# letitiabanana/PnP-OVSS

Measured on AMD Instinct MI355X. Metric: images/sec (336^2, drop_iter=4, blur+CRF), higher is better.
Workload: dtype bf16x3

## Files before the change

pnp-ovss_amd/csrc/engine.hip:

```cpp
#include <cmath>
#include <cstring>
#include <utility>

#include "engine.h"

using namespace pnp;

namespace {

int alloc_act(pnp_engine* e, Act* a, size_t rows, size_t ld) {
    KCHK(e, dalloc_t(e, &a->hi, rows * ld));
    a->lo = e->x3 ? (char*)a->hi + rows * ld * 2 : nullptr;
    return PNP_OK;
}

bool ends_with(const std::string& s, const char* suf) {
    const size_t n = strlen(suf);
    return s.size() >= n && s.compare(s.size() - n, n, suf) == 0;
}

__global__ void transpose_cast_kernel_f32(const float* __restrict__ in, float* __restrict__ out, int rows, int cols) {
    __shared__ float t[32][33];
    const int bx = blockIdx.x * 32, by = blockIdx.y * 32;
    for (int i = threadIdx.y; i < 32; i += 8) {
        const int r = by + i, c = bx + threadIdx.x;
        t[i][threadIdx.x] = (r < rows && c < cols) ? in[(size_t)r * cols + c] : 0.f;
    }
    __syncthreads();
    for (int i = threadIdx.y; i < 32; i += 8) {
        const int c = bx + i, r = by + threadIdx.x;
        if (r < rows && c < cols) out[(size_t)c * rows + r] = t[threadIdx.x][i];
    }
}

__global__ void feat_to_tok_kernel(const float* __restrict__ src, int ld_src, int n_pad, float* __restrict__ dst, int R, int N) {
    __shared__ float t[32][33];
    const int b = blockIdx.z, r0 = blockIdx.x * 32, t0 = blockIdx.y * 32;
    for (int i = threadIdx.y; i < 32; i += 8) {
        const int r = r0 + i, tok = t0 + threadIdx.x;
        t[i][threadIdx.x] = (r < R && tok < N) ? src[(size_t)r * ld_src + (size_t)b * n_pad + tok] : 0.f;
    }
    __syncthreads();
    for (int i = threadIdx.y; i < 32; i += 8) {
        const int tok = t0 + i, r = r0 + threadIdx.x;
        if (r < R && tok < N) dst[((size_t)b * N + tok) * R + r] = t[threadIdx.x][i];
    }
}
__global__ void tok_to_feat_kernel(const float* __restrict__ src, int ld_src, float* __restrict__ dst, int ld_dst, int n_pad, int R, int N) {
    __shared__ float t[32][33];
    const int b = blockIdx.z, r0 = blockIdx.x * 32, t0 = blockIdx.y * 32;
    for (int i = threadIdx.y; i < 32; i += 8) {
        const int tok = t0 + i, r = r0 + threadIdx.x;
        t[i][threadIdx.x] = (r < R && tok < N) ? src[((size_t)b * N + tok) * ld_src + r] : 0.f;
    }
    __syncthreads();
    for (int i = threadIdx.y; i < 32; i += 8) {
        const int r = r0 + i, tok = t0 + threadIdx.x;
        if (r < R && tok < N) dst[(size_t)r * ld_dst + (size_t)b * n_pad + tok] = t[threadIdx.x][i];
    }
}

__global__ void embed_reuse_kernel(const float* __restrict__ x0, const uint8_t* __restrict__ dropped, const float* __restrict__ bias,
                                   const float* __restrict__ pos, float* __restrict__ x, int rows, int N, int D4) {
    const size_t total = (size_t)rows * D4;
    for (size_t i = (size_t)blockIdx.x * blockDim.x + threadIdx.x; i < total; i += (size_t)gridDim.x * blockDim.x) {
        const int m = (int)(i / D4), c = (int)(i - (size_t)m * D4);
        const int b = m / N, t = m - b * N;
        f32x4 v;
        if (t > 0 && dropped[(size_t)b * (N - 1) + (t - 1)]) {
            const f32x4 bv = reinterpret_cast<const f32x4*>(bias)[c];
            const f32x4 pv = reinterpret_cast<const f32x4*>(pos)[(size_t)t * D4 + c];
#pragma unroll
            for (int e = 0; e < 4; e++) v[e] = __fadd_rn(__fadd_rn(0.0f, bv[e]), pv[e]);
        } else {
            v = reinterpret_cast<const f32x4*>(x0)[i];
        }
        reinterpret_cast<f32x4*>(x)[i] = v;
    }
}

int new_weight(pnp_engine* e, int rows, int cols, bool pair, Weight* w) {
    *w = Weight{nullptr, rows, cols, pair ? 2 : (int)e->esz, pair};
    return dalloc_t(e, &w->p, (size_t)rows * cols);
}
int fill_weight(pnp_engine* e, const float* src32, const Weight& w, int r0, int n) {
    const size_t count = (size_t)n * w.cols;
    return w.pair ? split_f32(src32, w.hi(r0), w.lo(r0), count, 0) : cast_f32(e->bf, src32, w.hi(r0), count, 0);
}
int make_weight(pnp_engine* e, const float* src32, int rows, int cols, bool transpose, Weight* out, bool pair = false) {
    KCHK(e, new_weight(e, transpose ? cols : rows, transpose ? rows : cols, pair, out));
    const float* s = src32;
    float* tmp = nullptr;
// ... 448 lines not shown
            KCHK(e, make_weight(e, st[W_SO], H, H, true, &t.so_wT, e->x3));
        }
    }
    for (int i = 0; i < 2; i++) {
        const float *w = staged(e, std::string(kProj[i]) + ".weight"), *bs = staged(e, std::string(kProj[i]) + ".bias");
        if (!w || !bs) {
            e->proj_E[i] = 0;
            continue;
        }
        KCHK(e, make_weight(e, w, e->proj_E[i], i == 0 ? D : H, false, &e->proj_w[i], e->x3));
        KCHK(e, dalloc(e, &e->proj_b[i], (size_t)e->proj_E[i]));
        HIPCHK(e, hipMemcpy(e->proj_b[i], bs, (size_t)e->proj_E[i] * 4, hipMemcpyDeviceToDevice));
    }
    HIPCHK(e, hipDeviceSynchronize());
    for (auto& b : e->staging) if (b.p) (void)hipFree(b.p);
    e->staging.clear();
    for (auto it = e->named.begin(); it != e->named.end();) {
        if (it->first.rfind("stage:", 0) == 0) it = e->named.erase(it);
        else ++it;
    }
    e->finalized = true;
    return PNP_OK;
}


static int vit_forward_impl(pnp_engine* e, const float* d_images, const uint8_t* d_dropped, int32_t B, void* stream, int embed) {
    if (!e || !d_images) return PNP_ERR_ARG;
    if (!e->finalized) return fail(e, PNP_ERR_STATE, "weights not finalized");
    if (B <= 0 || B > e->c.max_batch) return fail(e, PNP_ERR_ARG, "batch %d out of range (max %d)", B, e->c.max_batch);
    hipStream_t s = (hipStream_t)stream;
    const int D = e->D, N = e->N, M = B * N, F = D * e->c.vit_mlp_ratio, bf = e->bf;
    const int ldv = e->c.max_batch * e->Npad;
    if (embed == 2 && !(e->reuse.vit && e->reuse.images == d_images && e->reuse.B == B)) embed = 0;
    if (embed == 2 && d_dropped) {
        hipLaunchKernelGGL(embed_reuse_kernel, dim3(2048), dim3(256), 0, s, (const float*)e->x0, d_dropped, (const float*)e->patch_b,
                           (const float*)e->pos, e->x, M, N, D / 4);
        KCHK(e, launched());
    } else {
        KCHK(e, patchify(bf, d_images, d_dropped, e->patches, B, e->c.img_size, e->P, s));
        KCHK(e, cls_rows(e->cls, e->pos, e->x, B, N, D, s));
        {
            GemmArgs g = linear(e->patches, 768, e->patch_w, B * e->PP);
            g.bias = e->patch_b; g.resid = e->pos; g.ldr = D; g.out_f32 = e->x; g.ldo = D; g.row_div = e->PP;
            KCHK(e, egemm(e, g, s));
        }
        if (embed == 1) {
            HIPCHK(e, hipMemcpyAsync(e->x0, e->x, (size_t)M * D * sizeof(float), hipMemcpyDeviceToDevice, s));
            e->reuse.images = d_images;
            e->reuse.B = B;
            e->reuse.vit = true;
        }
    }
    const float scale = 1.0f / sqrtf(64.f);
    const int ln = bf | e->x3;
    for (int l = 0; l < e->c.vit_depth; l++) {
        const VitLayerW& w = e->vit[l];
        KCHK(e, layernorm(ln, e->x, w.n1w, w.n1b, e->c.vit_ln_eps, M, D, nullptr, e->xn.hi, nullptr, nullptr, s, e->xn.lo));
        if (bf || e->x3) {
            GemmArgs g = linear(e->xn, D, w.qkv_w, M);
            g.bias = w.qkv_b; g.out_t = e->qk.hi; g.out_lo = e->qk.lo; g.ldo_t = e->ldq;
            KCHK(e, egemm(e, g, s));
            if (e->x3)
                KCHK(e, vit_attention_x3(e->qk.hi, e->qk.lo, e->ldq, D, e->ctx.hi, e->ctx.lo, B, e->c.vit_heads, N, scale, s));
            else
                KCHK(e, vit_attention(bf, e->qk.hi, e->ldq, D, (const char*)e->qk.hi + (size_t)2 * D * e->esz, e->ldq, e->Npad, e->ctx.hi,
                                      B, e->c.vit_heads, N, scale, s));
        } else {
            {
                GemmArgs g = linear(e->xn, D, w.qkv_w, M, 0, 2 * D);
                g.bias = w.qkv_b; g.out_t = e->qk.hi; g.ldo_t = 2 * D;
                KCHK(e, egemm(e, g, s));
            }
            {
                GemmArgs g = linear_t(e->xn, D, w.qkv_w, M, 2 * D, D);
                g.bias = w.qkv_b + 2 * D; g.bias_on_rows = 1; g.out_t = e->vt; g.ldo_t = ldv; g.col_div = N; g.col_pad = e->Npad;
                KCHK(e, egemm(e, g, s));
            }
            KCHK(e, vit_attention(bf, e->qk.hi, 2 * D, D, e->vt, ldv, e->Npad, e->ctx.hi, B, e->c.vit_heads, N, scale, s));
        }
        {
            GemmArgs g = linear(e->ctx, D, w.proj_w, M);
            g.bias = w.proj_b; g.resid = e->x; g.ldr = D; g.out_f32 = e->x; g.ldo = D;
            KCHK(e, egemm(e, g, s));
        }
        KCHK(e, layernorm(ln, e->x, w.n2w, w.n2b, e->c.vit_ln_eps, M, D, nullptr, e->xn.hi, nullptr, nullptr, s, e->xn.lo));
        {
            GemmArgs g = linear(e->xn, D, w.fc1_w, M);
            g.bias = w.fc1_b; g.mode = GEMM_EPI_GELU; g.out_t = e->h1.hi; g.out_lo = e->h1.lo; g.ldo_t = F;
            KCHK(e, egemm(e, g, s));
        }
        {
            GemmArgs g = linear(e->h1, F, w.fc2_w, M);
            g.bias = w.fc2_b; g.resid = e->x; g.ldr = D; g.out_f32 = e->x; g.ldo = D;
            KCHK(e, egemm(e, g, s));
        }
    }
    KCHK(e, layernorm(ln, e->x, e->vnorm_w, e->vnorm_b, e->c.vit_ln_eps, M, D, e->emb32, e->embT.hi, nullptr, nullptr, s, e->embT.lo));
    return pnp_cross_kv(e, B, stream);
}
extern "C" int pnp_vit_forward(pnp_engine* e, const float* d_images, const uint8_t* d_dropped, int32_t B, void* stream) {
    if (e) e->reuse.vit = false;
    return vit_forward_impl(e, d_images, d_dropped, B, stream, 0);
}

extern "C" int pnp_cross_kv(pnp_engine* e, int32_t B, void* stream) {
    if (!e) return PNP_ERR_ARG;
    if (!e->finalized) return fail(e, PNP_ERR_STATE, "weights not finalized");
    if (B <= 0 || B > e->c.max_batch) return fail(e, PNP_ERR_ARG, "batch %d out of range (max %d)", B, e->c.max_batch);
    hipStream_t s = (hipStream_t)stream;
    const int D = e->D, N = e->N, M = B * N;
    const int ldv = e->c.max_batch * e->Npad;
    const int H = e->H, TL = e->TL, SL = e->SL, nVn = TL - SL, nKt = TL - SL - 1;
    auto out = [&](GemmArgs& g, void* p, int ld) {
        if (e->x3) { g.out_f32 = (float*)p; g.ldo = ld; }
        else { g.out_t = p; g.ldo_t = ld; }
    };
    {
        GemmArgs g = linear(e->embT, D, e->ck_w, M);
        g.bias = e->ck_b; out(g, e->Knat, TL * H);
        KCHK(e, egemm(e, g, s));
    }
    {
        GemmArgs g = linear_t(e->embT, D, e->cv_w, M);
        g.bias = e->cv_b; g.bias_on_rows = 1; out(g, e->Vt, ldv); g.col_div = N; g.col_pad = e->Npad;
        KCHK(e, egemm(e, g, s));
    }
    if (e->x3) {
        hipLaunchKernelGGL(feat_to_tok_kernel, dim3((nVn * H + 31) / 32, (N + 31) / 32, B), dim3(32, 8), 0, s,
                           (const float*)e->Vt + (size_t)SL * H * ldv, ldv, e->Npad, (float*)e->Vnat, nVn * H, N);
        KCHK(e, launched());
        if (nKt > 0) {
            hipLaunchKernelGGL(tok_to_feat_kernel, dim3((nKt * H + 31) / 32, (N + 31) / 32, B), dim3(32, 8), 0, s,
                               (const float*)e->Knat + (size_t)(SL + 1) * H, TL * H, (float*)e->Kt, ldv, e->Npad, nKt * H, N);
            KCHK(e, launched());
        }
        return PNP_OK;
    }
    {
        GemmArgs g = linear(e->embT, D, e->cv_w, M, SL * H, nVn * H);
        g.bias = e->cv_b + (size_t)SL * H; g.out_t = e->Vnat; g.ldo_t = nVn * H;
        KCHK(e, egemm(e, g, s));
    }
    if (nKt > 0) {
        GemmArgs g = linear_t(e->embT, D, e->ck_w, M, (SL + 1) * H, nKt * H);
        g.bias = e->ck_b + (size_t)(SL + 1) * H; g.bias_on_rows = 1; g.out_t = e->Kt; g.ldo_t = ldv; g.col_div = N; g.col_pad = e->Npad;
        KCHK(e, egemm(e, g, s));
    }
    return PNP_OK;
}

static int text_layer(pnp_engine* e, int i, const int64_t* d_mask, int32_t ld, int32_t B, int32_t L, bool cross, bool self_in_place,
                      hipStream_t s) {
    const int H = e->H, I = e->I, TL = e->TL, R = B * L, bf = e->bf, N = e->N;
    const int ldv = e->c.max_batch * e->Npad;
    const TextLayerW& w = e->txt[i];
    TextLayerA& a = e->ta[i];
    const float* h = i ? e->ta[i - 1].h_out : e->h0;
    const void* hT = i ? e->ta[i - 1].h_outT : e->h0T;
    const bool keep_p = cross && i >= e->SL;
    auto keep = [&](float* p) -> float* { return cross ? p : nullptr; };
    if (!self_in_place) {
        {
            GemmArgs g = linear(hT, H, w.qkv_w, R);
            g.bias = w.qkv_b; g.out_t = a.qkv; g.ldo_t = 3 * H;
            KCHK(e, egemm(e, g, s));
        }
// ... 264 lines not shown
    if (!e || !d_images || !d_ids || !d_mask || !d_g0) return PNP_ERR_ARG;
    if (drop_iter < 1) return fail(e, PNP_ERR_ARG, "drop_iter must be >= 1");
    if (drop_iter == 1)
        return pnp_compute_gradcam_layer(e, d_images, nullptr, d_ids, d_mask, ld, B, L, layer, head, d_g0, d_logits, stream);
    if (!d_agg || !d_picks) return PNP_ERR_ARG;
    hipStream_t s = (hipStream_t)stream;
    HIPCHK(e, hipMemsetAsync(e->dropped, 0, (size_t)B * e->PP, s));
    for (int it = 0; it < drop_iter; it++) {
        int r = compute_gradcam_impl(e, d_images, e->dropped, d_ids, d_mask, ld, B, L, layer, head, e->G, d_logits, stream, it == 0 ? 1 : 2);
        if (r) return r;
        r = pnp_drop_step(e, e->G, d_g0, d_agg, e->dropped, d_picks, it, B, L - 1, npick, drop_iter * npick, stream);
        if (r) return r;
    }
    return PNP_OK;
}


extern "C" int pnp_get_buffer(pnp_engine* e, const char* name, void** d_ptr, size_t* bytes) {
    if (!e || !name || !d_ptr || !bytes) return PNP_ERR_ARG;
    const std::string n(name);
    const size_t B = e->c.max_batch, L = e->c.max_text_len;
    auto set = [&](void* ptr, size_t b) { *d_ptr = ptr; *bytes = b; return PNP_OK; };
    if (n == "image_embeds") return set(e->emb32, B * e->N * (size_t)e->D * 4);
    if (n == "image_embeds_t") return set(e->embT.hi, B * e->N * (size_t)e->D * e->esz);
    if (n == "x") return set(e->x, B * e->N * (size_t)e->D * 4);
    if (n == "P") return set(e->ta[e->grad_layer >= 0 ? e->grad_layer : e->SL].Pc, B * e->nh * L * (size_t)e->Nst * 4);
    if (n == "dP") return set(e->dPc, B * e->nh * L * (size_t)e->Nst * 4);
    if (n == "text_hidden") return set(e->ta[e->TL - 1].h_out, B * L * (size_t)e->H * 4);
    if (n == "h_last") return set(e->ta[e->TL - 1].h_out, B * L * (size_t)e->H * 4);
    if (n == "dropped") return set(e->dropped, B * (size_t)e->PP);
    if (n == "P_last" && e->ta[e->TL - 1].Pc) return set(e->ta[e->TL - 1].Pc, B * e->nh * L * (size_t)e->Nst * 4);
    if (n == "Kt" && e->Kt) return set(e->Kt, (size_t)(e->TL - e->SL - 1) * e->H * B * e->Npad * e->esz);
    if (n == "Vt") return set(e->Vt, (size_t)e->TL * e->H * B * e->Npad * e->esz);
    if (n == "dq_xattn") return set(e->dqc, B * L * (size_t)e->H * e->esz);
    if (n == "dctx_xattn") return set(e->dctxc, B * L * (size_t)e->H * e->esz);
    if (post_get_buffer(e, n, d_ptr, bytes)) return PNP_OK;
    return fail(e, PNP_ERR_ARG, "unknown buffer %s", name);
}

extern "C" size_t pnp_allocated_bytes(const pnp_engine* e) { return e ? e->alloc_bytes : 0; }

extern "C" int pnp_profile_enable(pnp_engine* e, int32_t on) {
    if (!e) return PNP_ERR_ARG;
    if (!e->gemm_prof) {
        if (!on) {
            e->crf_prof.on = false;
            return PNP_OK;
        }
        e->gemm_prof = new GemmProfile();
    }
    GemmProfile& pf = *e->gemm_prof;
    pf.on = on != 0;
    pf.period = on > 1 ? on : 1;
    pf.seq = 0;
    pf.used = 0;
    pf.launches = 0;
    pf.flops = 0;
    e->crf_prof.on = on != 0;
    e->crf_prof.used = 0;
    e->crf_prof.launches = 0;
    e->crf_prof.work = 0;
    e->crf_prof.lattice = 0;
    return PNP_OK;
}

extern "C" int pnp_profile_read_stage(pnp_engine* e, int32_t stage, int64_t* launches, double* work, double* ms) {
// ... 48 lines not shown
                              void* d_out_t, int32_t ldo_t, int32_t mode, void* stream) {
    GemmArgs g = G_(d_A, lda, d_B, ldb, M, N, K);
    g.bias = d_bias; g.resid = d_resid; g.ldr = ldr; g.out_f32 = d_out_f32; g.ldo = ldo; g.out_t = d_out_t; g.ldo_t = ldo_t;
    g.mode = mode ? GEMM_EPI_GELU : GEMM_EPI_LINEAR;
    return gemm_nt(bf, g, (hipStream_t)stream);
}

extern "C" int pnp_op_split(const float* d_in, void* d_hi, void* d_lo, int64_t n, void* stream) {
    if (!d_in || !d_hi || !d_lo || n <= 0) return PNP_ERR_ARG;
    return split_f32(d_in, d_hi, d_lo, (size_t)n, (hipStream_t)stream);
}

extern "C" int pnp_op_gemm_x3(const void* d_A_hi, const void* d_A_lo, int32_t lda, const void* d_B_hi, const void* d_B_lo,
                              int32_t ldb, int32_t M, int32_t N, int32_t K, const float* d_bias, int32_t bias_on_rows,
                              const float* d_resid, int32_t ldr, float* d_out_f32, int32_t ldo, void* d_out_hi, void* d_out_lo,
                              int32_t ldo_t, int32_t gelu, int32_t col_div, int32_t col_pad, void* stream) {
    if (!d_A_hi || !d_A_lo || !d_B_hi || !d_B_lo) return PNP_ERR_ARG;
    GemmArgs g = G_(d_A_hi, lda, d_B_hi, ldb, M, N, K);
    g.A_lo = d_A_lo; g.B_lo = d_B_lo;
    g.bias = d_bias; g.bias_on_rows = bias_on_rows; g.resid = d_resid; g.ldr = ldr; g.out_f32 = d_out_f32; g.ldo = ldo;
    g.out_t = d_out_hi; g.out_lo = d_out_lo; g.ldo_t = ldo_t; g.col_div = col_div; g.col_pad = col_pad;
    g.mode = gelu ? GEMM_EPI_GELU : GEMM_EPI_LINEAR;
    g.sk = streamk_mode() ? streamk_ws_default() : nullptr;
    return gemm_nt(1, g, (hipStream_t)stream);
}

extern "C" int pnp_set_tuning(const char* key, int32_t value) {
    if (!key) return PNP_ERR_ARG;
    if (!strcmp(key, "streamk")) {
        if (value < 0 || value > 2) return PNP_ERR_ARG;
        set_streamk_mode(value);
        return PNP_OK;
    }
    if (!strcmp(key, "text_rows")) {
        if (value < 0 || value > 4) return PNP_ERR_ARG;
        set_text_rows(value);
        return PNP_OK;
    }
    if (!strcmp(key, "gemm_stamps")) {
        if (value < 0 || value > 1) return PNP_ERR_ARG;
        return gemm_set_stamps(value);
    }
    return PNP_ERR_ARG;
}

extern "C" int pnp_streamk_status(pnp_engine* e, int64_t* launches, uint32_t* gave_up) {
    if (!launches || !gave_up) return PNP_ERR_ARG;
    StreamKWs* ws = e ? &e->sk_ws : streamk_ws_default();
    *launches = ws ? ws->launches : 0;
    *gave_up = 0;
    if (!ws || !ws->part) return PNP_OK;
    if (e) HIPCHK(e, hipSetDevice(e->c.device));
    if (hipDeviceSynchronize() != hipSuccess) return PNP_ERR_HIP;
    return streamk_ws_timeouts(ws, gave_up);
}

extern "C" int pnp_op_gemm_x3a(const float* d_A, int32_t lda, const void* d_B_hi, const void* d_B_lo, int32_t ldb, int32_t M,
                               int32_t N, int32_t K, const float* d_bias, const float* d_resid, int32_t ldr, float* d_out_f32,
                               int32_t ldo, int32_t mode, float* d_aux, int32_t ld_aux, void* stream) {
    if (!d_A || !d_B_hi || !d_B_lo || !d_out_f32 || mode < 0 || mode > 2) return PNP_ERR_ARG;
    GemmArgs g = G_(d_A, lda, d_B_hi, ldb, M, N, K);
    g.B_lo = d_B_lo; g.a_f32 = 1;
    g.bias = d_bias; g.resid = d_resid; g.ldr = ldr; g.out_f32 = d_out_f32; g.ldo = ldo;
    g.mode = mode; g.aux = d_aux; g.ld_aux = ld_aux;
    return gemm_nt(0, g, (hipStream_t)stream);
}
// ... 157 lines not shown
```

pnp-ovss_amd/csrc/kernels.h:

```cpp
#pragma once
#include <hip/hip_runtime.h>
#include <stdint.h>
#include <stddef.h>
#include "gemm.h"

namespace pnp {

struct PostDesc {
    int H, W, K, C, has_bg, pix0;
    int Kp;
    int G, Kg;
    size_t off;
    size_t qoff;
    size_t voff[2];
};

struct alignas(16) CrfEntry {
    uint32_t pixel;
    float w;
    float nr;
    uint32_t pad;
};

struct alignas(16) CrfNbr8 {
    int ia, id;
    int pa, pd;
    int aa, ad;
    int da, dd;
};

struct CrfLattice {
    int D1;
    int which;
    size_t cap;
    float* bary;
    uint32_t* vals;
    CrfEntry* ent;
    int* offset;
    int* seg_start;
    int* seg_lo;
    int* seg_hi;
    uint64_t* ukeys;
    int* idbase;
    int* n1;
    int* n2;
    CrfNbr8* nbr8;
};

int patchify(int bf, const float* img, const uint8_t* dropped, void* out, int B, int S, int P, hipStream_t s);
int cls_rows(const float* cls, const float* pos, float* x, int B, int N, int D, hipStream_t s);
int layernorm(int bf, const float* x, const float* w, const float* b, float eps, int rows, int D, float* y, void* yt,
              float* xhat, float* rstd, hipStream_t s, void* yt_lo = nullptr);
int vit_attention(int bf, const void* qk, int ld_qk, int D, const void* vt, int ld_vt, int Npad, void* ctx, int B,
                  int H, int N, float scale, hipStream_t s, void* ctx_lo = nullptr);

int vit_attention_x3(const void* qkv_hi, const void* qkv_lo, int ld_qk, int D, void* ctx_hi, void* ctx_lo, int B, int H, int N,
                     float scale, hipStream_t s);

int text_embed(const int64_t* ids, int ld_ids, const float* word, const float* pos, float* out, int B, int L, int H,
               int enc_id, int vocab, hipStream_t s);
int text_self_attn(int bf, const void* qkv, const int64_t* mask, int ld_mask, void* ctx, float* probs, float* scratch, int B, int L,
                   int H, hipStream_t s);
void set_text_rows(int n);
int text_self_attn_bwd(int bf, const void* qkv, const float* dctx, const float* probs, float* ds_scratch, void* dqkv,
                       int B, int L, int H, hipStream_t s);
int xattn(int bf, int mode, const void* a1, int ld1, const void* a2t, int ld2, int Npad, const void* x, int ldx,
          void* out, int ldo, float* pbuf, int Nst, int B, int L, int N, int nheads, hipStream_t s);
int layernorm_bwd(int bf, const float* dy, const float* w, const float* xhat, const float* rstd, int rows, int D,
                  float* dx, void* dxt, hipStream_t s);
int itm_head(const float* hlast, const float* w, const float* bias, float* logits, int B, int L, int H, hipStream_t s);
int itm_grad_seed(const float* w, float* dh, int B, int L, int H, hipStream_t s);
int cast_f32(int bf, const float* in, void* out, size_t n, hipStream_t s);
int split_f32(const float* in, void* hi, void* lo, size_t n, hipStream_t s);

int l2_normalize_rows(float* x, int rows, int E, float eps, hipStream_t s);
int itc_similarity(const float* img, const float* txt, float* sim, int B, int T, int E, hipStream_t s);
int cast_rows_bf16(const float* in, int ld_in, void* out, int rows, int K, hipStream_t s);

int gradcam_gather(const float* P, const float* dP, const int64_t* mask, int ld_mask, float* out, int B, int nheads,
                   int head, int L, int Nst, int PP, hipStream_t s);
int drop_step(const float* G, float* g0, float* agg, uint8_t* dropped, int32_t* picks, int iter, int B, int T, int PP,
              int npick, int max_picks, hipStream_t s);
int merge_tokens(const float* src, const int32_t* cls_off, const int32_t* tok_idx, const int32_t* cls_div,
                 const int32_t* img_cls_off, float* out, int B, int T, int PP, int Cmax, hipStream_t s);
int threshold_maps(const float* merged, const int32_t* img_cls_off, float* out, float threshold, int B, int PP, int Cmax,
                   hipStream_t s);
int upsample_maps(const float* src, const PostDesc* desc, float* maps, int B, int P, int Cmax, int maxHW, hipStream_t s);
int minmax_normalize(float* maps, const PostDesc* desc, float* stats, int B, int Kmax, int maxHW, int class_channels_only,
                     hipStream_t s);
int background_channel(float* maps, const PostDesc* desc, int B, int maxHW, hipStream_t s);
// ... 69 lines not shown
```

pnp-ovss_amd/csrc/vit_kernels.hip:

```cpp
#include "common.h"
#include "kernels.h"

namespace pnp {

template <typename T>
__global__ void patchify_kernel(const float* __restrict__ img, const uint8_t* __restrict__ dropped,
                                T* __restrict__ out, int B, int S, int P) {
    const int idx = blockIdx.x * blockDim.x + threadIdx.x;
    const int total = B * P * P * 3 * 16;
    if (idx >= total) return;
    const int i = idx & 15;
    const int c = (idx >> 4) % 3;
    const int m = idx / 48;
    const int b = m / (P * P), p = m - b * P * P;
    const int py = p / P, px = p - py * P;
    T* o = out + (size_t)m * 768 + c * 256 + i * 16;
    const bool drop = dropped && dropped[m];
    const float* src = img + (((size_t)b * 3 + c) * S + (py * 16 + i)) * S + px * 16;
#pragma unroll
    for (int v = 0; v < 4; v++) {
        f32x4 x = drop ? f32x4{0.f, 0.f, 0.f, 0.f} : *reinterpret_cast<const f32x4*>(src + v * 4);
#pragma unroll
        for (int e = 0; e < 4; e++) o[v * 4 + e] = from_f32<T>(x[e]);
    }
}

__global__ void cls_rows_kernel(const float* __restrict__ cls, const float* __restrict__ pos,
                                float* __restrict__ x, int B, int N, int D) {
    const int idx = blockIdx.x * blockDim.x + threadIdx.x;
    if (idx >= B * D) return;
    const int b = idx / D, d = idx - b * D;
    x[(size_t)b * N * D + d] = cls[d] + pos[d];
// ... 168 lines not shown
                Frag<T> fv;
                lds_frag_acc_order<ROWB>(fv, Vs, dt * 16 + r, u, q);
                mma16(acc_o[dt], fv, fp);
            }
        }
    }
#undef PNP_LOAD_TILE
    if (q_valid) {
        const float inv = 1.0f / l_run;
        T* o = ctx + (row0 + qrow) * D + h * 64 + q * 4;
#pragma unroll
        for (int dt = 0; dt < 4; dt++) {
            if constexpr (sizeof(T) == 2) {
                bf16x4 pk = {(bf16)(acc_o[dt][0] * inv), (bf16)(acc_o[dt][1] * inv), (bf16)(acc_o[dt][2] * inv),
                             (bf16)(acc_o[dt][3] * inv)};
                *reinterpret_cast<bf16x4*>(o + dt * 16) = pk;
            } else {
                f32x4 ov = acc_o[dt] * inv;
                if (ctx_hi) {
                    const size_t off = (row0 + qrow) * D + h * 64 + q * 4 + dt * 16;
                    const bf16x4 ph = {(bf16)ov[0], (bf16)ov[1], (bf16)ov[2], (bf16)ov[3]};
                    const bf16x4 pl = {(bf16)(ov[0] - (float)ph[0]), (bf16)(ov[1] - (float)ph[1]), (bf16)(ov[2] - (float)ph[2]),
                                       (bf16)(ov[3] - (float)ph[3])};
                    *reinterpret_cast<bf16x4*>(ctx_hi + off) = ph;
                    *reinterpret_cast<bf16x4*>(ctx_lo + off) = pl;
                } else {
                    *reinterpret_cast<f32x4*>(o + dt * 16) = ov;
                }
            }
        }
    }
}

__global__ __launch_bounds__(512) void vit_attn32_kernel(const bf16* __restrict__ qk, int ld_qk, int D,
                                                         const bf16* __restrict__ vt, int ld_vt, int Npad,
                                                         bf16* __restrict__ ctx, int N, float scale, int nqw) {
    constexpr int ROWB = 128, TILE = 64 * ROWB;
    __shared__ __attribute__((aligned(16))) char ring[2][2 * TILE];

    const int tid = threadIdx.x, lane = tid & 63, wave = __builtin_amdgcn_readfirstlane(tid >> 6);
    const int nwaves = blockDim.x >> 6;
    const int l32 = lane & 31, hi = lane >> 5;
    const int b = blockIdx.z, h = blockIdx.y;
    const size_t row0 = (size_t)b * N;
    const int qw = blockIdx.x * nwaves + wave;
    int qrow = qw * 32 + l32;
    const bool q_valid = qw < nqw && qrow < N;
    qrow = qrow < N ? qrow : N - 1;

    bf16x8 fq[4];
    {
        const bf16* qp = qk + (row0 + qrow) * ld_qk + h * 64 + hi * 8;
#pragma unroll
        for (int ks = 0; ks < 4; ks++) fq[ks] = *reinterpret_cast<const bf16x8*>(qp + ks * 16);
    }

    const char* kbase = reinterpret_cast<const char*>(qk + row0 * ld_qk + D + h * 64);
    const char* vbase = reinterpret_cast<const char*>(vt + row0 * ld_vt + h * 64);
    const int prow = lane >> 3, pc = lane & 7;
    auto issue_tile = [&](int t) {
        char* dst = ring[t & 1];
        for (int p = wave; p < 16; p += nwaves) {
            const int row = (p & 7) * 8 + prow;
            const int sc = pc ^ ((row >> 1) & 7);
            int key = t * 64 + row;
            key = key < N ? key : N - 1;
            const char* src = p < 8 ? kbase + (size_t)key * ld_qk * 2 + sc * 16 : vbase + (size_t)key * ld_vt * 2 + sc * 16;
            __builtin_amdgcn_global_load_lds((const __attribute__((address_space(1))) void*)src,
                                             (__attribute__((address_space(3))) void*)(dst + p * 1024), 16, 0, 0);
        }
    };

    f32x16 o[2];
#pragma unroll
    for (int i = 0; i < 2; i++)
#pragma unroll
        for (int e = 0; e < 16; e++) o[i][e] = 0.f;
    float m_run = -INFINITY, l_run = 0.f;
// ... 64 lines not shown
#pragma unroll
            for (int dt = 0; dt < 2; dt++) {
                typedef __attribute__((ext_vector_type(4))) short s16x4;
                s16x4 part[2];
#pragma unroll
                for (int u = 0; u < 2; u++) {
                    const int key = 16 * j + 8 * u + 4 * hi + tq;
                    const int col = dt * 32 + grp_d + 4 * tp;
                    const char* a = Vs + key * ROWB + ((((col >> 3)) ^ ((key >> 1) & 7)) << 4) + (col & 7) * 2;
                    part[u] = __builtin_amdgcn_ds_read_tr16_b64_v4i16((__attribute__((address_space(3))) s16x4*)a);
                }
                const bf16x4 lo = __builtin_bit_cast(bf16x4, part[0]), hh = __builtin_bit_cast(bf16x4, part[1]);
                const bf16x8 fv = {lo[0], lo[1], lo[2], lo[3], hh[0], hh[1], hh[2], hh[3]};
                o[dt] = __builtin_amdgcn_mfma_f32_32x32x16_bf16(fv, fp[j], o[dt], 0, 0, 0);
            }
    }
    l_run += __shfl_xor(l_run, 32, 64);
    if (q_valid) {
        const float inv = 1.0f / l_run;
        bf16* op = ctx + (row0 + qrow) * D + h * 64 + hi * 4;
#pragma unroll
        for (int dt = 0; dt < 2; dt++)
#pragma unroll
            for (int g4 = 0; g4 < 4; g4++) {
                const bf16x4 pk = {(bf16)(o[dt][g4 * 4] * inv), (bf16)(o[dt][g4 * 4 + 1] * inv), (bf16)(o[dt][g4 * 4 + 2] * inv),
                                   (bf16)(o[dt][g4 * 4 + 3] * inv)};
                *reinterpret_cast<bf16x4*>(op + dt * 32 + g4 * 8) = pk;
            }
    }
}

__global__ __launch_bounds__(768) void vit_attn32_x3_kernel(const bf16* __restrict__ qk, const bf16* __restrict__ qk_lo, int ld_qk, int D,
                                                            const bf16* __restrict__ vt, const bf16* __restrict__ vt_lo, int ld_vt,
                                                            bf16* __restrict__ ctx, bf16* __restrict__ ctx_lo, int N, float scale, int nqw) {
    constexpr int ROWB = 128, TILE = 64 * ROWB;
    __shared__ __attribute__((aligned(16))) char ring[2][4 * TILE];

    const int tid = threadIdx.x, lane = tid & 63, wave = __builtin_amdgcn_readfirstlane(tid >> 6);
    const int nwaves = blockDim.x >> 6;
    const int l32 = lane & 31, hi = lane >> 5;
    const int b = blockIdx.z, h = blockIdx.y;
    const size_t row0 = (size_t)b * N;
    const int qw = blockIdx.x * nwaves + wave;
    int qrow = qw * 32 + l32;
    const bool q_valid = qw < nqw && qrow < N;
    qrow = qrow < N ? qrow : N - 1;

    bf16x8 fq[4], fql[4];
    {
        const size_t off = (row0 + qrow) * ld_qk + h * 64 + hi * 8;
#pragma unroll
        for (int ks = 0; ks < 4; ks++) {
            fq[ks] = *reinterpret_cast<const bf16x8*>(qk + off + ks * 16);
            fql[ks] = *reinterpret_cast<const bf16x8*>(qk_lo + off + ks * 16);
        }
    }
    const size_t koff = (row0 * ld_qk + D + h * 64) * 2, voff = (row0 * ld_vt + h * 64) * 2;
    const uint64_t k0 = reinterpret_cast<uint64_t>(qk) + koff;
    const uint64_t d_klo = reinterpret_cast<uint64_t>(qk_lo) + koff - k0;
    const uint64_t d_v = reinterpret_cast<uint64_t>(vt) + voff - k0;
    const uint64_t d_vlo = reinterpret_cast<uint64_t>(vt_lo) + voff - k0;
    const int prow = lane >> 3, pc = lane & 7;
    const uint32_t sc_even = (uint32_t)(pc ^ ((prow >> 1) & 7)) << 4, sc_odd = (uint32_t)(pc ^ ((4 + (prow >> 1)) & 7)) << 4;
    auto issue_tile = [&](int t) {
        for (int p = wave; p < 32; p += nwaves) {
            const uint64_t m_v = 0ull - (uint64_t)((p >> 3) & 1), m_lo = 0ull - (uint64_t)(p >> 4);
            const uint64_t d = (m_v & m_lo & d_vlo) | (m_v & ~m_lo & d_v) | (~m_v & m_lo & d_klo);
            const uint32_t ld2 = ((uint32_t)ld_qk + ((uint32_t)m_v & (uint32_t)(ld_vt - ld_qk))) * 2u;
            int rs = t * 64 + (p & 7) * 8;
            rs = rs < N - 1 ? rs : N - 1;
            const char* const sbase = reinterpret_cast<const char*>(k0 + d + (uint64_t)((uint32_t)rs * ld2));
            int lr = rs + prow;
            lr = (lr < N ? lr : N - 1) - rs;
            const uint32_t loff = (uint32_t)lr * ld2 + ((p & 1) ? sc_odd : sc_even);
            const uint32_t lds = (uint32_t)(uintptr_t)(__attribute__((address_space(3))) char*)(ring[t & 1] + p * 1024);
            const uint64_t sb = reinterpret_cast<uint64_t>(sbase);
// ... 91 lines not shown
                        const int col = dt * 32 + grp_d + 4 * tp;
                        const char* a = V + key * ROWB + ((((col >> 3)) ^ ((key >> 1) & 7)) << 4) + (col & 7) * 2;
                        pr[u] = __builtin_amdgcn_ds_read_tr16_b64_v4i16((__attribute__((address_space(3))) s16x4*)a);
                    }
                    const bf16x4 lo = __builtin_bit_cast(bf16x4, pr[0]), hh = __builtin_bit_cast(bf16x4, pr[1]);
                    fv[part] = bf16x8{lo[0], lo[1], lo[2], lo[3], hh[0], hh[1], hh[2], hh[3]};
                }
                o[dt] = __builtin_amdgcn_mfma_f32_32x32x16_bf16(fv[1], fp[j], o[dt], 0, 0, 0);
                o[dt] = __builtin_amdgcn_mfma_f32_32x32x16_bf16(fv[0], fpl[j], o[dt], 0, 0, 0);
                o[dt] = __builtin_amdgcn_mfma_f32_32x32x16_bf16(fv[0], fp[j], o[dt], 0, 0, 0);
            }
    }
    l_run += __shfl_xor(l_run, 32, 64);
    if (q_valid) {
        const float inv = 1.0f / l_run;
        const size_t off = (row0 + qrow) * D + h * 64 + hi * 4;
#pragma unroll
        for (int dt = 0; dt < 2; dt++)
#pragma unroll
            for (int g4 = 0; g4 < 4; g4++) {
                bf16x4 ph, pl;
#pragma unroll
                for (int e = 0; e < 4; e++) {
                    const float v = o[dt][g4 * 4 + e] * inv;
                    ph[e] = (bf16)v;
                    pl[e] = (bf16)(v - (float)ph[e]);
                }
                *reinterpret_cast<bf16x4*>(ctx + off + dt * 32 + g4 * 8) = ph;
                *reinterpret_cast<bf16x4*>(ctx_lo + off + dt * 32 + g4 * 8) = pl;
            }
    }
}

int vit_attention(int bf, const void* qk, int ld_qk, int D, const void* vt, int ld_vt, int Npad, void* ctx, int B,
                  int H, int N, float scale, hipStream_t s, void* ctx_lo) {
    if (D != H * 64 || Npad % 64 || Npad < N) return PNP_ERR_ARG;
    if (bf) {
        if (ctx_lo) return PNP_ERR_ARG;
        const int nqw = (N + 31) / 32;
        const int max_wpb = 8;
        const int nblk = (nqw + max_wpb - 1) / max_wpb, wpb = (nqw + nblk - 1) / nblk;
        hipLaunchKernelGGL(vit_attn32_kernel, dim3(nblk, H, B), dim3(wpb * 64), 0, s, (const bf16*)qk, ld_qk, D,
                           (const bf16*)vt, ld_vt, Npad, (bf16*)ctx, N, scale, nqw);
        return hipGetLastError() == hipSuccess ? PNP_OK : PNP_ERR_HIP;
    }
    dim3 grid((N + 63) / 64, H, B);
    hipLaunchKernelGGL((vit_attn_kernel<float>), grid, dim3(256), 0, s, (const float*)qk, ld_qk, D, (const float*)vt, ld_vt,
                       Npad, ctx_lo ? nullptr : (float*)ctx, N, scale, ctx_lo ? (bf16*)ctx : nullptr, (bf16*)ctx_lo);
    return hipGetLastError() == hipSuccess ? PNP_OK : PNP_ERR_HIP;
}

int vit_attention_x3(const void* qkv_hi, const void* qkv_lo, int ld_qk, int D, void* ctx_hi, void* ctx_lo, int B, int H, int N,
                     float scale, hipStream_t s) {
    if (D != H * 64 || !qkv_hi || !qkv_lo || !ctx_hi || !ctx_lo) return PNP_ERR_ARG;
    const int nqw = (N + 31) / 32;
    const int max_wpb = nqw > 24 ? 12 : 8;
    const int nblk = (nqw + max_wpb - 1) / max_wpb, wpb = (nqw + nblk - 1) / nblk;
    const bf16 *qh = (const bf16*)qkv_hi, *ql = (const bf16*)qkv_lo;
    hipLaunchKernelGGL(vit_attn32_x3_kernel, dim3(nblk, H, B), dim3(wpb * 64), 0, s, qh, ql, ld_qk, D, qh + 2 * D, ql + 2 * D, ld_qk,
                       (bf16*)ctx_hi, (bf16*)ctx_lo, N, scale, nqw);
    return hipGetLastError() == hipSuccess ? PNP_OK : PNP_ERR_HIP;
}

int patchify(int bf, const float* img, const uint8_t* dropped, void* out, int B, int S, int P, hipStream_t s) {
    const int total = B * P * P * 48;
    const int nb = (total + 255) / 256;
    if (bf) hipLaunchKernelGGL((patchify_kernel<bf16>), dim3(nb), dim3(256), 0, s, img, dropped, (bf16*)out, B, S, P);
    else hipLaunchKernelGGL((patchify_kernel<float>), dim3(nb), dim3(256), 0, s, img, dropped, (float*)out, B, S, P);
    return hipGetLastError() == hipSuccess ? PNP_OK : PNP_ERR_HIP;
}

int cls_rows(const float* cls, const float* pos, float* x, int B, int N, int D, hipStream_t s) {
    hipLaunchKernelGGL(cls_rows_kernel, dim3((B * D + 255) / 256), dim3(256), 0, s, cls, pos, x, B, N, D);
    return hipGetLastError() == hipSuccess ? PNP_OK : PNP_ERR_HIP;
}

int layernorm(int bf, const float* x, const float* w, const float* b, float eps, int rows, int D, float* y, void* yt,
              float* xhat, float* rstd, hipStream_t s, void* yt_lo) {
    if (D > 1024 || D % 4) return PNP_ERR_ARG;
    if (yt_lo && !bf) return PNP_ERR_ARG;
    const int nb = (rows + 3) / 4;
    if (bf) hipLaunchKernelGGL((layernorm_kernel<bf16>), dim3(nb), dim3(256), 0, s, x, w, b, eps, rows, D, y, (bf16*)yt, xhat, rstd, (bf16*)yt_lo);
    else hipLaunchKernelGGL((layernorm_kernel<float>), dim3(nb), dim3(256), 0, s, x, w, b, eps, rows, D, y, (float*)yt, xhat, rstd, (bf16*)nullptr);
    return hipGetLastError() == hipSuccess ? PNP_OK : PNP_ERR_HIP;
}

}
```

Measured before the change: 219.0.

## Vectorize feature/token transposes, drop embed copy, remap attention grid for pairing

```diff
diff --git a/pnp-ovss_amd/csrc/engine.hip b/pnp-ovss_amd/csrc/engine.hip
--- a/pnp-ovss_amd/csrc/engine.hip
+++ b/pnp-ovss_amd/csrc/engine.hip
@@ -33,31 +33,53 @@
     }
 }
 
-__global__ void feat_to_tok_kernel(const float* __restrict__ src, int ld_src, int n_pad, float* __restrict__ dst, int R, int N) {
-    __shared__ float t[32][33];
-    const int b = blockIdx.z, r0 = blockIdx.x * 32, t0 = blockIdx.y * 32;
-    for (int i = threadIdx.y; i < 32; i += 8) {
-        const int r = r0 + i, tok = t0 + threadIdx.x;
-        t[i][threadIdx.x] = (r < R && tok < N) ? src[(size_t)r * ld_src + (size_t)b * n_pad + tok] : 0.f;
+__device__ __forceinline__ void transpose_tile64(const float* __restrict__ src, size_t ld_s, float* __restrict__ dst, size_t ld_d,
+                                                 int ni, int nj, bool vec) {
+    __shared__ float t[64][65];
+    const int tid = threadIdx.x;
+    const bool wide = vec && ni >= 64 && nj >= 64;
+    const int q = tid & 15, w16 = tid >> 4;
+    const int c = tid & 63, w4 = tid >> 6;
+    if (wide) {
+        f32x4 v[4];
+#pragma unroll
+        for (int k = 0; k < 4; k++) v[k] = *reinterpret_cast<const f32x4*>(src + (size_t)(w16 + 16 * k) * ld_s + 4 * q);
+#pragma unroll
+        for (int k = 0; k < 4; k++)
+#pragma unroll
+            for (int e = 0; e < 4; e++) t[w16 + 16 * k][4 * q + e] = v[k][e];
+    } else {
+        for (int i = w4; i < 64; i += 4) t[i][c] = (i < ni && c < nj) ? src[(size_t)i * ld_s + c] : 0.f;
     }
     __syncthreads();
-    for (int i = threadIdx.y; i < 32; i += 8) {
-        const int tok = t0 + i, r = r0 + threadIdx.x;
-        if (r < R && tok < N) dst[((size_t)b * N + tok) * R + r] = t[threadIdx.x][i];
-    }
-}
-__global__ void tok_to_feat_kernel(const float* __restrict__ src, int ld_src, float* __restrict__ dst, int ld_dst, int n_pad, int R, int N) {
-    __shared__ float t[32][33];
-    const int b = blockIdx.z, r0 = blockIdx.x * 32, t0 = blockIdx.y * 32;
-    for (int i = threadIdx.y; i < 32; i += 8) {
-        const int tok = t0 + i, r = r0 + threadIdx.x;
-        t[i][threadIdx.x] = (r < R && tok < N) ? src[((size_t)b * N + tok) * ld_src + r] : 0.f;
-    }
-    __syncthreads();
-    for (int i = threadIdx.y; i < 32; i += 8) {
-        const int r = r0 + i, tok = t0 + threadIdx.x;
-        if (r < R && tok < N) dst[(size_t)r * ld_dst + (size_t)b * n_pad + tok] = t[threadIdx.x][i];
-    }
+    if (wide) {
+#pragma unroll
+        for (int k = 0; k < 4; k++) {
+            const int j = w16 + 16 * k;
+            f32x4 o;
+#pragma unroll
+            for (int e = 0; e < 4; e++) o[e] = t[4 * q + e][j];
+            *reinterpret_cast<f32x4*>(dst + (size_t)j * ld_d + 4 * q) = o;
+        }
+    } else {
+        for (int j = w4; j < 64; j += 4)
+            if (j < nj && c < ni) dst[(size_t)j * ld_d + c] = t[c][j];
+    }
+}
+__global__ __launch_bounds__(256) void feat_to_tok_kernel(const float* __restrict__ src, int ld_src, int n_pad, float* __restrict__ dst,
+                                                          int R, int N, int vec) {
+    const int b = blockIdx.z, r0 = blockIdx.x * 64, t0 = blockIdx.y * 64;
+    transpose_tile64(src + (size_t)r0 * ld_src + (size_t)b * n_pad + t0, ld_src, dst + ((size_t)b * N + t0) * R + r0, R,
+                     min(64, R - r0), min(64, N - t0), vec);
+}
+__global__ __launch_bounds__(256) void tok_to_feat_kernel(const float* __restrict__ src, int ld_src, float* __restrict__ dst, int ld_dst,
+                                                          int n_pad, int R, int N, int vec) {
+    const int b = blockIdx.z, r0 = blockIdx.x * 64, t0 = blockIdx.y * 64;
+    transpose_tile64(src + ((size_t)b * N + t0) * ld_src + r0, ld_src, dst + (size_t)r0 * ld_dst + (size_t)b * n_pad + t0, ld_dst,
+                     min(64, N - t0), min(64, R - r0), vec);
+}
+bool tiles_aligned16(const void* src, const void* dst, int ld_a, int ld_b, int n_pad) {
+    return !(((uintptr_t)src | (uintptr_t)dst) & 15) && !((ld_a | ld_b | n_pad) & 3);
 }
 
 __global__ void embed_reuse_kernel(const float* __restrict__ x0, const uint8_t* __restrict__ dropped, const float* __restrict__ bias,
@@ -572,20 +594,21 @@
     const int D = e->D, N = e->N, M = B * N, F = D * e->c.vit_mlp_ratio, bf = e->bf;
     const int ldv = e->c.max_batch * e->Npad;
     if (embed == 2 && !(e->reuse.vit && e->reuse.images == d_images && e->reuse.B == B)) embed = 0;
+    float* x_in = e->x;
     if (embed == 2 && d_dropped) {
         hipLaunchKernelGGL(embed_reuse_kernel, dim3(2048), dim3(256), 0, s, (const float*)e->x0, d_dropped, (const float*)e->patch_b,
                            (const float*)e->pos, e->x, M, N, D / 4);
         KCHK(e, launched());
     } else {
+        if (embed == 1) x_in = e->x0;
         KCHK(e, patchify(bf, d_images, d_dropped, e->patches, B, e->c.img_size, e->P, s));
-        KCHK(e, cls_rows(e->cls, e->pos, e->x, B, N, D, s));
+        KCHK(e, cls_rows(e->cls, e->pos, x_in, B, N, D, s));
         {
             GemmArgs g = linear(e->patches, 768, e->patch_w, B * e->PP);
-            g.bias = e->patch_b; g.resid = e->pos; g.ldr = D; g.out_f32 = e->x; g.ldo = D; g.row_div = e->PP;
+            g.bias = e->patch_b; g.resid = e->pos; g.ldr = D; g.out_f32 = x_in; g.ldo = D; g.row_div = e->PP;
             KCHK(e, egemm(e, g, s));
         }
         if (embed == 1) {
-            HIPCHK(e, hipMemcpyAsync(e->x0, e->x, (size_t)M * D * sizeof(float), hipMemcpyDeviceToDevice, s));
             e->reuse.images = d_images;
             e->reuse.B = B;
             e->reuse.vit = true;
@@ -595,7 +618,8 @@
     const int ln = bf | e->x3;
     for (int l = 0; l < e->c.vit_depth; l++) {
         const VitLayerW& w = e->vit[l];
-        KCHK(e, layernorm(ln, e->x, w.n1w, w.n1b, e->c.vit_ln_eps, M, D, nullptr, e->xn.hi, nullptr, nullptr, s, e->xn.lo));
+        const float* x_l = l ? e->x : x_in;
+        KCHK(e, layernorm(ln, x_l, w.n1w, w.n1b, e->c.vit_ln_eps, M, D, nullptr, e->xn.hi, nullptr, nullptr, s, e->xn.lo));
         if (bf || e->x3) {
             GemmArgs g = linear(e->xn, D, w.qkv_w, M);
             g.bias = w.qkv_b; g.out_t = e->qk.hi; g.out_lo = e->qk.lo; g.ldo_t = e->ldq;
@@ -620,7 +644,7 @@
         }
         {
             GemmArgs g = linear(e->ctx, D, w.proj_w, M);
-            g.bias = w.proj_b; g.resid = e->x; g.ldr = D; g.out_f32 = e->x; g.ldo = D;
+            g.bias = w.proj_b; g.resid = x_l; g.ldr = D; g.out_f32 = e->x; g.ldo = D;
             KCHK(e, egemm(e, g, s));
         }
         KCHK(e, layernorm(ln, e->x, w.n2w, w.n2b, e->c.vit_ln_eps, M, D, nullptr, e->xn.hi, nullptr, nullptr, s, e->xn.lo));
@@ -665,13 +689,15 @@
         g.bias = e->cv_b; g.bias_on_rows = 1; out(g, e->Vt, ldv); g.col_div = N; g.col_pad = e->Npad;
         KCHK(e, egemm(e, g, s));
     }
-    if (e->x3) {
-        hipLaunchKernelGGL(feat_to_tok_kernel, dim3((nVn * H + 31) / 32, (N + 31) / 32, B), dim3(32, 8), 0, s,
-                           (const float*)e->Vt + (size_t)SL * H * ldv, ldv, e->Npad, (float*)e->Vnat, nVn * H, N);
+    if (e->esz == 4) {
+        const float* vsrc = (const float*)e->Vt + (size_t)SL * H * ldv;
+        hipLaunchKernelGGL(feat_to_tok_kernel, dim3((nVn * H + 63) / 64, (N + 63) / 64, B), dim3(256), 0, s, vsrc, ldv, e->Npad,
+                           (float*)e->Vnat, nVn * H, N, (int)tiles_aligned16(vsrc, e->Vnat, ldv, nVn * H, e->Npad));
         KCHK(e, launched());
         if (nKt > 0) {
-            hipLaunchKernelGGL(tok_to_feat_kernel, dim3((nKt * H + 31) / 32, (N + 31) / 32, B), dim3(32, 8), 0, s,
-                               (const float*)e->Knat + (size_t)(SL + 1) * H, TL * H, (float*)e->Kt, ldv, e->Npad, nKt * H, N);
+            const float* ksrc = (const float*)e->Knat + (size_t)(SL + 1) * H;
+            hipLaunchKernelGGL(tok_to_feat_kernel, dim3((nKt * H + 63) / 64, (N + 63) / 64, B), dim3(256), 0, s, ksrc, TL * H,
+                               (float*)e->Kt, ldv, e->Npad, nKt * H, N, (int)tiles_aligned16(ksrc, e->Kt, TL * H, ldv, e->Npad));
             KCHK(e, launched());
         }
         return PNP_OK;
@@ -1002,6 +1028,8 @@
     if (n == "P_last" && e->ta[e->TL - 1].Pc) return set(e->ta[e->TL - 1].Pc, B * e->nh * L * (size_t)e->Nst * 4);
     if (n == "Kt" && e->Kt) return set(e->Kt, (size_t)(e->TL - e->SL - 1) * e->H * B * e->Npad * e->esz);
     if (n == "Vt") return set(e->Vt, (size_t)e->TL * e->H * B * e->Npad * e->esz);
+    if (n == "Knat") return set(e->Knat, B * e->N * (size_t)e->TL * e->H * e->esz);
+    if (n == "Vnat") return set(e->Vnat, B * e->N * (size_t)(e->TL - e->SL) * e->H * e->esz);
     if (n == "dq_xattn") return set(e->dqc, B * L * (size_t)e->H * e->esz);
     if (n == "dctx_xattn") return set(e->dctxc, B * L * (size_t)e->H * e->esz);
     if (post_get_buffer(e, n, d_ptr, bytes)) return PNP_OK;
@@ -1116,6 +1144,11 @@
         set_streamk_mode(value);
         return PNP_OK;
     }
+    if (!strcmp(key, "attn_pairing")) {
+        if (value < 0 || value > 1) return PNP_ERR_ARG;
+        set_attn_pairing(value);
+        return PNP_OK;
+    }
     if (!strcmp(key, "text_rows")) {
         if (value < 0 || value > 4) return PNP_ERR_ARG;
         set_text_rows(value);
diff --git a/pnp-ovss_amd/csrc/kernels.h b/pnp-ovss_amd/csrc/kernels.h
--- a/pnp-ovss_amd/csrc/kernels.h
+++ b/pnp-ovss_amd/csrc/kernels.h
@@ -56,6 +56,7 @@
 
 int vit_attention_x3(const void* qkv_hi, const void* qkv_lo, int ld_qk, int D, void* ctx_hi, void* ctx_lo, int B, int H, int N,
                      float scale, hipStream_t s);
+void set_attn_pairing(int on);
 
 int text_embed(const int64_t* ids, int ld_ids, const float* word, const float* pos, float* out, int B, int L, int H,
                int enc_id, int vocab, hipStream_t s);
diff --git a/pnp-ovss_amd/csrc/vit_kernels.hip b/pnp-ovss_amd/csrc/vit_kernels.hip
--- a/pnp-ovss_amd/csrc/vit_kernels.hip
+++ b/pnp-ovss_amd/csrc/vit_kernels.hip
@@ -1,3 +1,5 @@
+#include <atomic>
+
 #include "common.h"
 #include "kernels.h"
 
@@ -232,18 +234,36 @@
     }
 }
 
+__device__ __forceinline__ bool attn_workgroup(int pairing, int nblk, int H, int npairs, int& part, int& h, int& b) {
+    const int L = blockIdx.x;
+    int pair;
+    if (pairing) {
+        const int i = L >> 3;
+        part = i % nblk;
+        pair = (i / nblk) * 8 + (L & 7);
+    } else {
+        part = L % nblk;
+        pair = L / nblk;
+    }
+    h = pair % H;
+    b = pair / H;
+    return pair < npairs;
+}
+
 __global__ __launch_bounds__(512) void vit_attn32_kernel(const bf16* __restrict__ qk, int ld_qk, int D,
                                                          const bf16* __restrict__ vt, int ld_vt, int Npad,
-                                                         bf16* __restrict__ ctx, int N, float scale, int nqw) {
+                                                         bf16* __restrict__ ctx, int N, float scale, int nqw, int nblk, int H,
+                                                         int npairs, int pairing) {
     constexpr int ROWB = 128, TILE = 64 * ROWB;
     __shared__ __attribute__((aligned(16))) char ring[2][2 * TILE];
 
     const int tid = threadIdx.x, lane = tid & 63, wave = __builtin_amdgcn_readfirstlane(tid >> 6);
     const int nwaves = blockDim.x >> 6;
     const int l32 = lane & 31, hi = lane >> 5;
-    const int b = blockIdx.z, h = blockIdx.y;
+    int part, h, b;
+    if (!attn_workgroup(pairing, nblk, H, npairs, part, h, b)) return;
     const size_t row0 = (size_t)b * N;
-    const int qw = blockIdx.x * nwaves + wave;
+    const int qw = part * nwaves + wave;
     int qrow = qw * 32 + l32;
     const bool q_valid = qw < nqw && qrow < N;
     qrow = qrow < N ? qrow : N - 1;
@@ -374,16 +394,18 @@
 
 __global__ __launch_bounds__(768) void vit_attn32_x3_kernel(const bf16* __restrict__ qk, const bf16* __restrict__ qk_lo, int ld_qk, int D,
                                                             const bf16* __restrict__ vt, const bf16* __restrict__ vt_lo, int ld_vt,
-                                                            bf16* __restrict__ ctx, bf16* __restrict__ ctx_lo, int N, float scale, int nqw) {
+                                                            bf16* __restrict__ ctx, bf16* __restrict__ ctx_lo, int N, float scale, int nqw,
+                                                            int nblk, int H, int npairs, int pairing) {
     constexpr int ROWB = 128, TILE = 64 * ROWB;
     __shared__ __attribute__((aligned(16))) char ring[2][4 * TILE];
 
     const int tid = threadIdx.x, lane = tid & 63, wave = __builtin_amdgcn_readfirstlane(tid >> 6);
     const int nwaves = blockDim.x >> 6;
     const int l32 = lane & 31, hi = lane >> 5;
-    const int b = blockIdx.z, h = blockIdx.y;
+    int part, h, b;
+    if (!attn_workgroup(pairing, nblk, H, npairs, part, h, b)) return;
     const size_t row0 = (size_t)b * N;
-    const int qw = blockIdx.x * nwaves + wave;
+    const int qw = part * nwaves + wave;
     int qrow = qw * 32 + l32;
     const bool q_valid = qw < nqw && qrow < N;
     qrow = qrow < N ? qrow : N - 1;
@@ -541,6 +563,10 @@
     }
 }
 
+static std::atomic<int> g_attn_pairing{1};
+void set_attn_pairing(int on) { g_attn_pairing.store(on, std::memory_order_relaxed); }
+static dim3 attn_grid(int pairing, int nblk, int npairs) { return dim3((pairing ? (npairs + 7) / 8 * 8 : npairs) * nblk); }
+
 int vit_attention(int bf, const void* qk, int ld_qk, int D, const void* vt, int ld_vt, int Npad, void* ctx, int B,
                   int H, int N, float scale, hipStream_t s, void* ctx_lo) {
     if (D != H * 64 || Npad % 64 || Npad < N) return PNP_ERR_ARG;
@@ -549,8 +575,9 @@
         const int nqw = (N + 31) / 32;
         const int max_wpb = 8;
         const int nblk = (nqw + max_wpb - 1) / max_wpb, wpb = (nqw + nblk - 1) / nblk;
-        hipLaunchKernelGGL(vit_attn32_kernel, dim3(nblk, H, B), dim3(wpb * 64), 0, s, (const bf16*)qk, ld_qk, D,
-                           (const bf16*)vt, ld_vt, Npad, (bf16*)ctx, N, scale, nqw);
+        const int pairing = g_attn_pairing.load(std::memory_order_relaxed);
+        hipLaunchKernelGGL(vit_attn32_kernel, attn_grid(pairing, nblk, H * B), dim3(wpb * 64), 0, s, (const bf16*)qk, ld_qk, D,
+                           (const bf16*)vt, ld_vt, Npad, (bf16*)ctx, N, scale, nqw, nblk, H, H * B, pairing);
         return hipGetLastError() == hipSuccess ? PNP_OK : PNP_ERR_HIP;
     }
     dim3 grid((N + 63) / 64, H, B);
@@ -566,8 +593,9 @@
     const int max_wpb = nqw > 24 ? 12 : 8;
     const int nblk = (nqw + max_wpb - 1) / max_wpb, wpb = (nqw + nblk - 1) / nblk;
     const bf16 *qh = (const bf16*)qkv_hi, *ql = (const bf16*)qkv_lo;
-    hipLaunchKernelGGL(vit_attn32_x3_kernel, dim3(nblk, H, B), dim3(wpb * 64), 0, s, qh, ql, ld_qk, D, qh + 2 * D, ql + 2 * D, ld_qk,
-                       (bf16*)ctx_hi, (bf16*)ctx_lo, N, scale, nqw);
+    const int pairing = g_attn_pairing.load(std::memory_order_relaxed);
+    hipLaunchKernelGGL(vit_attn32_x3_kernel, attn_grid(pairing, nblk, H * B), dim3(wpb * 64), 0, s, qh, ql, ld_qk, D, qh + 2 * D,
+                       ql + 2 * D, ld_qk, (bf16*)ctx_hi, (bf16*)ctx_lo, N, scale, nqw, nblk, H, H * B, pairing);
     return hipGetLastError() == hipSuccess ? PNP_OK : PNP_ERR_HIP;
 }
 
```

Result: no change. 219.5 (median of 6 runs) (+0.2%).
